# mika314/melonix

Measured on AMD Instinct MI355X. Metric: STFT+pitch+resynth frames/sec (48 kHz, 4096 FFT, 256 hop); % HBM roofline, higher is better.
Workload: dtype f32

## Files before the change

### melonix_amd/csrc/stft_core.h

```cpp
#pragma once
#include <stdint.h>
#include <type_traits>

#if defined(__HIPCC__)
#include <hip/hip_runtime.h>
#define MX_HD __host__ __device__ __forceinline__
namespace mx {
using cpx = float2;
}
#else
#define MX_HD inline __attribute__((always_inline))
namespace mx {
struct alignas(8) cpx {
  float x, y;
};
}
#endif

namespace mx {

#include "stft_consts.inc"

MX_HD cpx mk(float x, float y) {
  cpx r;
  r.x = x;
  r.y = y;
  return r;
}
MX_HD float fma_(float a, float b, float c) { return __builtin_fmaf(a, b, c); }
MX_HD cpx cadd(cpx a, cpx b) { return mk(a.x + b.x, a.y + b.y); }
MX_HD cpx csub(cpx a, cpx b) { return mk(a.x - b.x, a.y - b.y); }
MX_HD cpx cmul(cpx a, cpx b) { return mk(fma_(a.x, b.x, -(a.y * b.y)), fma_(a.x, b.y, a.y * b.x)); }
MX_HD float cnorm2(cpx a) { return fma_(a.x, a.x, a.y * a.y); }
MX_HD cpx cconj(cpx a) { return mk(a.x, -a.y); }
MX_HD cpx csel(bool c, cpx a, cpx b) { return mk(c ? a.x : b.x, c ? a.y : b.y); }
MX_HD float fast_sqrt(float x) {
#if defined(__HIP_DEVICE_COMPILE__)
  return __builtin_amdgcn_sqrtf(x);
#else
  return __builtin_sqrtf(x);
#endif
}
MX_HD constexpr int ilog2(int x) { return x <= 1 ? 0 : 1 + ilog2(x >> 1); }

}
#include "pk_math.h"
namespace mx {

template <int K>
MX_HD cpx mulw64(cpx a) {
  constexpr int k = ((K % 64) + 64) % 64;
  constexpr float h = 0.707106781187f;
  if constexpr (k == 0) return a;
  else if constexpr (k == 16) return mk(a.y, -a.x);
  else if constexpr (k == 32) return mk(-a.x, -a.y);
  else if constexpr (k == 48) return mk(-a.y, a.x);
  else if constexpr (k == 8) return mk(h * (a.x + a.y), h * (a.y - a.x));
  else if constexpr (k == 24) return mk(h * (a.y - a.x), -h * (a.x + a.y));
  else if constexpr (k == 40) return mk(-h * (a.x + a.y), h * (a.x - a.y));
  else if constexpr (k == 56) return mk(h * (a.x - a.y), h * (a.x + a.y));
  else {
    constexpr float c = kCos64[k], s = kSin64[k];
    return mk(fma_(a.x, c, a.y * s), fma_(a.y, c, -(a.x * s)));
  }
}

template <int K>
MX_HD void bfly_w64(cpx E, cpx O, cpx &out0, cpx &out1) {
  constexpr int k = ((K % 64) + 64) % 64;
  if constexpr (k == 0) {
    pk_bfly_1(E, O, out0, out1);
  } else if constexpr (k == 16) {
    pk_bfly_mi(E, O, out0, out1);
  } else if constexpr (k == 32) {
    pk_bfly_1(E, O, out1, out0);
  } else if constexpr (k == 48) {
    pk_bfly_mi(E, O, out1, out0);
  } else {
    pk_bfly_cs(E, O, mk(kCos64[k], kSin64[k]), out0, out1);
  }
}

template <int R, int Q>
struct Combine {
  static MX_HD void run(const cpx *E, const cpx *O, cpx *out) {
    bfly_w64<Q * 64 / R>(E[Q], O[Q], out[Q], out[Q + R / 2]);
    if constexpr (Q + 1 < R / 2) Combine<R, Q + 1>::run(E, O, out);
  }
};

template <int R>
struct Dft {
  static MX_HD void run(const cpx *in, cpx *out) {
    cpx e[R / 2], o[R / 2], E[R / 2], O[R / 2];
#pragma unroll
    for (int q = 0; q < R / 2; ++q) {
      e[q] = in[2 * q];
      o[q] = in[2 * q + 1];
    }
    Dft<R / 2>::run(e, E);
    Dft<R / 2>::run(o, O);
    Combine<R, 0>::run(E, O, out);
  }
};
template <>
struct Dft<2> {
  static MX_HD void run(const cpx *in, cpx *out) {
    pk_bfly_1(in[0], in[1], out[0], out[1]);
  }
};
template <>
struct Dft<1> {
  static MX_HD void run(const cpx *in, cpx *out) { out[0] = in[0]; }
};

template <int R, int S, int O0, bool CONJ>
struct DftTw {
  static MX_HD void run(const cpx *v, const cpx *w, cpx *out) {
    if constexpr (R == 2) {
      constexpr int i0 = O0, i1 = O0 + S;
      if constexpr (i0 == 0) pk_leaf0_tw<CONJ>(v[0], v[i1], w[i1], out[0], out[1]);
      else pk_leaf_tw<CONJ>(v[i0], w[i0], v[i1], w[i1], out[0], out[1]);
    } else {
      cpx E[R / 2], O[R / 2];
      DftTw<R / 2, 2 * S, O0, CONJ>::run(v, w, E);
      DftTw<R / 2, 2 * S, O0 + S, CONJ>::run(v, w, O);
      Combine<R, 0>::run(E, O, out);
    }
  }
};

template <int N_, int E_>
struct Plan {
  static constexpr int N = N_;
  static constexpr int M = N / 2;
  static constexpr int E = E_;
  static constexpr int T = M / E;
  static constexpr int R3 = E / 2;
  static constexpr int R1 = (N == 4096) ? 16 : 32;
  static constexpr int R2 = M / (R1 * R3);
  static constexpr int NS3 = R1 * R2;
  static constexpr int NB1 = E / R1;
  static constexpr int NB2 = E / R2;
  static constexpr int TW2 = (R2 - 1) * R1;
  static constexpr int TW3 = (R3 - 1) * NS3;
  static constexpr int L1 = ilog2(R1);
  static_assert(N == 4096 || N == 16384 || N == 32768, "supported FFT sizes");
  static_assert((N == 4096) ? E == 16 : E == 32, "supported points per thread");
  static_assert(R1 * R2 * R3 == M && R2 <= E && R1 <= E && T % 64 == 0, "radix plan must cover M");
};

template <class P>
MX_HD constexpr bool t1_padded() { return P::R1 == 32; }
template <class P>
MX_HD constexpr int t1_size() { return t1_padded<P>() ? P::M + P::M / 32 : P::M; }
template <class P>
MX_HD int t1_index(int i) {
  if constexpr (t1_padded<P>()) return i + (i >> 5);
  else return i ^ ((i >> P::L1) & 15);
}

struct alignas(4) f2u {
  float x, y;
};
template <bool ALIGNED8>
MX_HD cpx ld_pair(const float *base, int i) {
  const char *a = reinterpret_cast<const char *>(base) + (size_t)(4u * (unsigned)i);
  if constexpr (ALIGNED8) {
    return *reinterpret_cast<const cpx *>(a);
  } else {
    const f2u u = *reinterpret_cast<const f2u *>(a);
    return mk(u.x, u.y);
  }
}

MX_HD float ld_one(const float *base, int i) {
  return *reinterpret_cast<const float *>(reinterpret_cast<const char *>(base) + (size_t)(4u * (unsigned)i));
}

template <class P, int WSTEP, bool ALIGNED8>
MX_HD void load_frame(int t, cpx (&Y)[P::E], const float *x, const float *w) {
#pragma unroll
  for (int e = 0; e < P::E; ++e) {
    const int p = 2 * (t + P::T * e);
    cpx xs, ws;
    if constexpr (ALIGNED8 && WSTEP == 1) {
      xs = ld_pair<true>(x, p);
      ws = ld_pair<true>(w, p);
    } else {
      xs = ld_pair<false>(x, p);
      if constexpr (WSTEP == 1) {
        ws = ld_pair<false>(w, p);
      } else {
        const f2u wu = *reinterpret_cast<const f2u *>(w - p - 1);
        ws = mk(wu.y, wu.x);
      }
    }
    Y[e] = pk_mul(xs, ws);
  }
}

template <int T>
MX_HD constexpr float win_grow(int e) {
  return T == 64 ? kWinGrow64[e] : T == 128 ? kWinGrow128[e] : T == 256 ? kWinGrow256[e] : kWinGrow512[e];
}
template <class P, bool CLAMP = true>
MX_HD cpx geo_weight(cpx a0, int e) {
  constexpr float sc = 0.5f / (float)P::N;
  const float g = e == 0 ? 1.0f : win_grow<P::T>(e);
  const cpx w = e == 0 ? a0 : mk(a0.x * g, a0.y * g);
  if constexpr (!CLAMP) {
    return w;
  } else {
    const unsigned sb = __builtin_bit_cast(unsigned, sc), xb = __builtin_bit_cast(unsigned, w.x), yb = __builtin_bit_cast(unsigned, w.y);
    return mk(__builtin_bit_cast(float, xb < sb ? xb : sb), __builtin_bit_cast(float, yb < sb ? yb : sb));
  }
}
template <class P>
MX_HD int geo_clamped_slots(int hop) { return (hop + 2 * P::T - 1) / (2 * P::T); }
constexpr int kGeoTail = 2;
template <class P, bool ALIGNED8>
MX_HD void load_frame_geo(int t, cpx (&Y)[P::E], const float *x, const float *wb, int hop) {
  static_assert(P::T == 64 || P::T == 128 || P::T == 256 || P::T == 512, "growth table per T");
  static_assert(P::E <= 32, "growth table length");
  const cpx a0 = ld_pair<true>(wb, 2 * t);
  if (geo_clamped_slots<P>(hop) <= kGeoTail) {
#pragma unroll
    for (int e = 0; e < P::E; ++e) {
      const cpx xs = ld_pair<ALIGNED8>(x, 2 * (t + P::T * e));
      Y[e] = pk_mul(xs, e < P::E - kGeoTail ? geo_weight<P, false>(a0, e) : geo_weight<P, true>(a0, e));
    }
  } else {
#pragma unroll
    for (int e = 0; e < P::E; ++e) Y[e] = pk_mul(ld_pair<ALIGNED8>(x, 2 * (t + P::T * e)), geo_weight<P, true>(a0, e));
  }
}

template <class P>
MX_HD void apply_window_geo(int t, cpx (&Y)[P::E], const cpx (&xr)[P::E], const float *wb, int hop) {
  const cpx a0 = ld_pair<true>(wb, 2 * t);
  if (geo_clamped_slots<P>(hop) <= kGeoTail) {
#pragma unroll
    for (int e = 0; e < P::E; ++e)
      Y[e] = pk_mul(xr[e], e < P::E - kGeoTail ? geo_weight<P, false>(a0, e) : geo_weight<P, true>(a0, e));
  } else {
#pragma unroll
    for (int e = 0; e < P::E; ++e) Y[e] = pk_mul(xr[e], geo_weight<P, true>(a0, e));
  }
}

template <class P, bool ALIGNED8>
MX_HD void load_raw(int t, cpx (&xr)[P::E], const float *x) {
#pragma unroll
  for (int e = 0; e < P::E; ++e) {
    xr[e] = ld_pair<ALIGNED8>(x, 2 * (t + P::T * e));
  }
}
template <class P, int WSTEP, bool ALIGNED8>
MX_HD void apply_window(int t, cpx (&Y)[P::E], const cpx (&xr)[P::E], const float *w) {
#pragma unroll
  for (int e = 0; e < P::E; ++e) {
    const int p = 2 * (t + P::T * e);
    cpx ws;
    if constexpr (WSTEP == 1) {
      ws = ld_pair<ALIGNED8>(w, p);
    } else {
      const f2u wu = *reinterpret_cast<const f2u *>(w - p - 1);
      ws = mk(wu.y, wu.x);
    }
    Y[e] = pk_mul(xr[e], ws);
  }
}

template <class P>
MX_HD void pass1(const cpx (&Y)[P::E], cpx (&v)[P::E]) {
#pragma unroll
  for (int b = 0; b < P::NB1; ++b) {
    cpx in[P::R1], out[P::R1];
#pragma unroll
    for (int r = 0; r < P::R1; ++r) in[r] = Y[b + P::NB1 * r];
    Dft<P::R1>::run(in, out);
#pragma unroll
    for (int r = 0; r < P::R1; ++r) v[b * P::R1 + r] = out[r];
  }
}

template <class P, int HOP>
struct Slide {
  static constexpr int H = HOP / 2;
  static constexpr bool ok = (HOP > 0) && (HOP % 2 == 0) && (H % P::T == 0) && (2 * (H / P::T) <= P::E);
  static constexpr int D = ok ? H / P::T : 1;
};

template <class P, int HOP>
MX_HD void slide_edge(int t, const float *wtab, float inv_sc, cpx (&edge)[Slide<P, HOP>::D]) {
  using S = Slide<P, HOP>;
#pragma unroll
  for (int i = 0; i < S::D; ++i) {
    const int p = 2 * (t + P::T * (P::E - 2 * S::D + i));
    edge[i] = mk(wtab[p] * inv_sc, wtab[p + 1] * inv_sc);
  }
}

template <class P, int HOP>
MX_HD void slide_fetch(int t, const float *xe, cpx (&nx)[Slide<P, HOP>::D]) {
  using S = Slide<P, HOP>;
#pragma unroll
  for (int i = 0; i < S::D; ++i) nx[i] = *reinterpret_cast<const cpx *>(xe - HOP + 2 * (t + P::T * i));
}

template <class P, int HOP>
MX_HD void slide_step(cpx (&Y)[P::E], const cpx (&nx)[Slide<P, HOP>::D], const cpx (&edge)[Slide<P, HOP>::D],
                      float g, float sc) {
  using S = Slide<P, HOP>;
  const cpx gg = mk(g, g), ss = mk(sc, sc);
#pragma unroll
  for (int e = 0; e < P::E - 2 * S::D; ++e) Y[e] = pk_mul_xs(Y[e + S::D], gg);
#pragma unroll
  for (int i = 0; i < S::D; ++i) Y[P::E - 2 * S::D + i] = pk_mul(Y[P::E - S::D + i], edge[i]);
#pragma unroll
  for (int i = 0; i < S::D; ++i) Y[P::E - S::D + i] = pk_mul_xs(nx[i], ss);
}


template <class P>
struct Circ {
  static constexpr int W = 2 * P::T;
  static constexpr int CS = (P::T == 128) ? 4 : (P::T == 256) ? 3 : 2;
  static MX_HD bool ok(int hop) { return hop >= 1 && hop <= (CS - 1) * P::T && hop <= 2 * W; }
  static constexpr int slot(int k) { return (P::E - (CS - 1) + k) & (P::E - 1); }
};
template <class P>
struct CircGeo {
  int o;
  int s;
  int cr;
  int len;
};
template <class P>
MX_HD CircGeo<P> circ_geo(long long frame_end, int hop) {
  constexpr int W = Circ<P>::W;
  const long long start = frame_end - P::N;
  CircGeo<P> g;
  g.o = (int)(start & (long long)(W - 1));
  g.s = ((int)((start - hop) & (long long)(W - 1)) + hop) / W;
  g.len = 2 * hop;
  g.cr = (g.o - g.len) & (P::N - 1);
  return g;
}
template <class P>
MX_HD void circ_load_first(int t, cpx (&Y)[P::E], const float *xa, const float *w, int o) {
#pragma unroll
  for (int e = 0; e < P::E; ++e) {
    const int c2 = 2 * (t + P::T * e);
    const int q0 = (c2 - o) & (P::N - 1), q1 = (c2 + 1 - o) & (P::N - 1);
    Y[e] = mk(xa[q0] * w[q0], xa[q1] * w[q1]);
  }
}
template <class P>
MX_HD void circ_fetch(int t, const float *xs, const float *wt, const CircGeo<P> &g, float (&px)[2 * Circ<P>::CS],
                      float (&pw)[2 * Circ<P>::CS]) {
#pragma unroll
  for (int k = 0; k < Circ<P>::CS; ++k) {
    const int c2 = 2 * (t + P::T * Circ<P>::slot(k));
    int d0 = (c2 - g.cr) & (P::N - 1), d1 = (c2 + 1 - g.cr) & (P::N - 1);
    d0 = d0 < g.len ? d0 : g.len - 1;
    d1 = d1 < g.len ? d1 : g.len - 1;
    px[2 * k] = ld_one(xs, d0);
    px[2 * k + 1] = ld_one(xs, d1);
    pw[2 * k] = ld_one(wt, d0);
    pw[2 * k + 1] = ld_one(wt, d1);
  }
}
template <class P, int S>
MX_HD void circ_age(cpx (&Y)[P::E], cpx gg) {
  cpx head[S > 0 ? S : 1];
#pragma unroll
  for (int i = 0; i < S; ++i) head[i] = Y[i];
#pragma unroll
  for (int e = 0; e < P::E - S; ++e) Y[e] = pk_mul_xs(Y[e + S], gg);
#pragma unroll
  for (int i = 0; i < S; ++i) Y[P::E - S + i] = pk_mul_xs(head[i], gg);
}
template <class P>
MX_HD void circ_step(int t, cpx (&Y)[P::E], float decay, const CircGeo<P> &g, const float (&px)[2 * Circ<P>::CS],
                     const float (&pw)[2 * Circ<P>::CS]) {
  const cpx gg = mk(decay, decay);
  constexpr int SMAX = (Circ<P>::W - 1 + (Circ<P>::CS - 1) * P::T) / Circ<P>::W;
  static_assert(SMAX <= 2, "rotations by 0, 1 or 2 slots");
  if (g.s == 0) circ_age<P, 0>(Y, gg);
  else if (SMAX == 1 || g.s == 1) circ_age<P, 1>(Y, gg);
  else circ_age<P, 2>(Y, gg);
#pragma unroll
  for (int k = 0; k < Circ<P>::CS; ++k) {
    const int e = Circ<P>::slot(k);
    const int c2 = 2 * (t + P::T * e);
    const int d0 = (c2 - g.cr) & (P::N - 1), d1 = (c2 + 1 - g.cr) & (P::N - 1);
    const float n0 = px[2 * k] * pw[2 * k], n1 = px[2 * k + 1] * pw[2 * k + 1];
    Y[e] = mk(d0 < g.len ? n0 : Y[e].x, d1 < g.len ? n1 : Y[e].y);
  }
}


#if defined(__HIP_DEVICE_COMPILE__)
#define MX_LDS_ASM 1
typedef float mx_f2v __attribute__((ext_vector_type(2)));
template <int OFF>
__device__ __forceinline__ mx_f2v lds_rd64(uint32_t addr) {
  static_assert(OFF >= 0 && OFF < 163840, "LDS is 160 KiB");
  mx_f2v r;
  if constexpr (OFF < 65536) {
    asm volatile("ds_read_b64 %0, %1 offset:%2" : "=v"(r) : "v"(addr), "n"(OFF) : "memory");
  } else {
    const uint32_t hi = addr + (uint32_t)(OFF & ~65535);
    asm volatile("ds_read_b64 %0, %1 offset:%2" : "=v"(r) : "v"(hi), "n"(OFF & 65535) : "memory");
  }
  return r;
}
__device__ __forceinline__ uint32_t lds_addr(const void *p) {
  return (uint32_t)(uintptr_t)(const __attribute__((address_space(3))) void *)p;
}
template <int N>
__device__ __forceinline__ void lds_wait(mx_f2v (&q)[N]) {
  static_assert(N % 8 == 0, "tied in groups of 8");
  asm volatile("s_waitcnt lgkmcnt(0)" ::: "memory");
#pragma unroll
  for (int i = 0; i < N; i += 8)
    asm volatile("" : "+v"(q[i]), "+v"(q[i + 1]), "+v"(q[i + 2]), "+v"(q[i + 3]), "+v"(q[i + 4]),
                 "+v"(q[i + 5]), "+v"(q[i + 6]), "+v"(q[i + 7]));
}
#endif
template <int I, int N, class F>
MX_HD void static_for(F &&f) {
  if constexpr (I < N) {
    f(std::integral_constant<int, I>{});
    static_for<I + 1, N>(f);
  }
}

template <class P>
MX_HD void store_t1(int t, const cpx (&v)[P::E], cpx *lds) {
  if constexpr (t1_padded<P>()) {
    static_assert(P::R1 <= 32 && (P::T * P::R1) % 32 == 0, "T1 padding is one point per 32");
    cpx *const p = lds + (t * P::R1 + ((t * P::R1) >> 5));
#pragma unroll
    for (int b = 0; b < P::NB1; ++b) {
#pragma unroll
      for (int r = 0; r < P::R1; ++r) p[b * (P::T * P::R1 + P::T * P::R1 / 32) + r] = v[b * P::R1 + r];
    }
  } else {
    const unsigned B8 = (unsigned)((t * P::R1) ^ (t & 15)) << 3;
    char *const base = reinterpret_cast<char *>(lds);
#pragma unroll
    for (int r = 0; r < P::R1; ++r) {
      cpx *p = reinterpret_cast<cpx *>(base + (B8 ^ ((unsigned)r << 3)));
#pragma unroll
      for (int b = 0; b < P::NB1; ++b) p[b * P::T * P::R1] = v[b * P::R1 + r];
    }
  }
}

template <class P>
struct T1Read {
  static constexpr int S = P::M / P::R2;
  static constexpr int SP = t1_padded<P>() ? S + S / 32 : S;
  static constexpr int TP = t1_padded<P>() ? P::T + P::T / 32 : P::T;
  static constexpr int step = t1_padded<P>() ? 0 : ((S >> P::L1) & 15);
  static_assert(S % 32 == 0 && P::T % 32 == 0 && (step == 0 || step == 8), "T1 read is base(+alt base) + offset");
  static_assert(t1_padded<P>() || P::NB2 == 1, "the XOR layout's bases are written for one pass-2 butterfly per thread");
};

template <class P>
MX_HD void load_t1(int t, cpx (&v)[P::E], const cpx *lds) {
  using R = T1Read<P>;
  const int s1 = t1_index<P>(t);
#ifdef MX_LDS_ASM
  mx_f2v q[P::E];
  const uint32_t ae = lds_addr(lds + s1), ao = lds_addr(lds + (s1 ^ R::step));
  static_for<0, P::NB2>([&](auto bb) {
    constexpr int b = decltype(bb)::value;
    static_for<0, P::R2>([&](auto rr) {
      constexpr int r = decltype(rr)::value;
      q[b * P::R2 + r] = lds_rd64<(b * R::TP + r * R::SP) * 8>((r & 1) ? ao : ae);
    });
  });
  lds_wait(q);
#pragma unroll
  for (int i = 0; i < P::E; ++i) v[i] = mk(q[i].x, q[i].y);
#else
  const cpx *pe = lds + s1, *po = lds + (s1 ^ R::step);
#pragma unroll
  for (int b = 0; b < P::NB2; ++b) {
#pragma unroll
    for (int r = 0; r < P::R2; ++r) v[b * P::R2 + r] = ((r & 1) ? po : pe)[b * R::TP + r * R::SP];
  }
#endif
}

template <class P>
MX_HD void load_t1_tw2(int t, cpx (&v)[P::E], const cpx *lds, const cpx *ltw2, cpx (&w)[P::R2 - 1]) {
  static_assert(P::NB2 == 1 && P::E == P::R2 && P::E % 8 == 0, "one pass-2 butterfly per thread");
  using R = T1Read<P>;
  const int s1 = t1_index<P>(t);
#ifdef MX_LDS_ASM
  const uint32_t ae = lds_addr(lds + s1), ao = lds_addr(lds + (s1 ^ R::step));
  const uint32_t aw = lds_addr(ltw2 + (t & (P::R1 - 1)));
  mx_f2v q[2 * P::E];
  static_for<0, P::R2>([&](auto rr) {
    constexpr int r = decltype(rr)::value;
    q[r] = lds_rd64<r * R::SP * 8>((r & 1) ? ao : ae);
  });
  static_for<1, P::R2>([&](auto rr) {
    constexpr int r = decltype(rr)::value;
    q[P::E + r] = lds_rd64<(r - 1) * P::R1 * 8>(aw);
  });
  q[P::E] = mx_f2v{0.0f, 0.0f};
  lds_wait(q);
#pragma unroll
  for (int i = 0; i < P::E; ++i) v[i] = mk(q[i].x, q[i].y);
#pragma unroll
  for (int r = 1; r < P::R2; ++r) w[r - 1] = mk(q[P::E + r].x, q[P::E + r].y);
#else
  const cpx *pe = lds + s1, *po = lds + (s1 ^ R::step), *pw = ltw2 + (t & (P::R1 - 1));
#pragma unroll
  for (int r = 0; r < P::R2; ++r) v[r] = ((r & 1) ? po : pe)[r * R::SP];
#pragma unroll
  for (int r = 1; r < P::R2; ++r) w[r - 1] = pw[(r - 1) * P::R1];
#endif
}

template <class P>
MX_HD void pass2(int t, cpx (&v)[P::E], const cpx *tw2) {
#pragma unroll
  for (int b = 0; b < P::NB2; ++b) {
    const int j = t + P::T * b;
    const int k = j & (P::R1 - 1);
    cpx in[P::R2], w[P::R2], out[P::R2];
    w[0] = mk(1.0f, 0.0f);
#pragma unroll
    for (int r = 0; r < P::R2; ++r) in[r] = v[b * P::R2 + r];
#pragma unroll
    for (int r = 1; r < P::R2; ++r) {
      w[r] = tw2[(r - 1) * P::R1 + k];
    }
    DftTw<P::R2, 1, 0, false>::run(in, w, out);
#pragma unroll
    for (int r = 0; r < P::R2; ++r) v[b * P::R2 + r] = out[r];
  }
}

template <class P>
MX_HD void pass2_reg(cpx (&v)[P::E], const cpx (&w)[P::R2 - 1]) {
  static_assert(P::NB2 == 1, "one pass-2 butterfly per thread");
  cpx in[P::R2], ww[P::R2], out[P::R2];
  ww[0] = mk(1.0f, 0.0f);
#pragma unroll
  for (int r = 0; r < P::R2; ++r) in[r] = v[r];
#pragma unroll
  for (int r = 1; r < P::R2; ++r) ww[r] = w[r - 1];
  DftTw<P::R2, 1, 0, false>::run(in, ww, out);
#pragma unroll
  for (int r = 0; r < P::R2; ++r) v[r] = out[r];
}

template <class P>
MX_HD void store_t2(int t, const cpx (&v)[P::E], cpx *lds) {
#pragma unroll
  for (int b = 0; b < P::NB2; ++b) {
    const int j = t + P::T * b;
    const int k = j & (P::R1 - 1);
    const int base = (j - k) * P::R2 + k;
    cpx *p = lds + base;
#pragma unroll
    for (int r = 0; r < P::R2; ++r) p[r * P::R1] = v[b * P::R2 + r];
  }
}

template <class P>
MX_HD int k0p(int t) { return t; }
template <class P>
MX_HD int k0q(int t) { return t ? P::NS3 - t : P::NS3 / 2; }

template <class P>
MX_HD void load_t2(int t, cpx (&v)[P::E], const cpx *lds) {
  const int p = k0p<P>(t), q = k0q<P>(t);
#ifdef MX_LDS_ASM
  {
    const uint32_t pa = lds_addr(lds + p), qa = lds_addr(lds + q);
    mx_f2v w[P::E];
    static_for<0, P::R3>([&](auto rr) {
      constexpr int r = decltype(rr)::value;
      w[r] = lds_rd64<P::NS3 * r * 8>(pa);
      w[P::R3 + r] = lds_rd64<P::NS3 * r * 8>(qa);
    });
    lds_wait(w);
#pragma unroll
    for (int i = 0; i < P::E; ++i) v[i] = mk(w[i].x, w[i].y);
  }
#else
  const cpx *pp = lds + p, *qq = lds + q;
#pragma unroll
  for (int r = 0; r < P::R3; ++r) {
    v[r] = pp[P::NS3 * r];
    v[P::R3 + r] = qq[P::NS3 * r];
  }
#endif
}

template <class P>
MX_HD constexpr int q_index(int r) { return P::R3 + ((r + 1) & (P::R3 - 1)); }

template <class P>
MX_HD void fetch_tw3(int t, const cpx *tw3, cpx (&w)[P::R3 - 1]) {
  const int col = t ? t : P::NS3 / 2;
#pragma unroll
  for (int r = 1; r < P::R3; ++r) w[r - 1] = tw3[(r - 1) * P::NS3 + col];
}
template <class P>
MX_HD void fetch_tw3_bases(int t, const cpx *tw3, cpx (&wb)[6]) {
  static_assert(P::R3 == 16, "two-level pass-3 twiddles are written for radix 16");
  const int col = t ? t : P::NS3 / 2;
  constexpr int rr[6] = {1, 2, 3, 4, 8, 12};
#pragma unroll
  for (int i = 0; i < 6; ++i) wb[i] = tw3[(rr[i] - 1) * P::NS3 + col];
}
template <class P, bool MAY0>
MX_HD void pass3_reg(int t, cpx (&v)[P::E], const cpx (&w)[P::R3 - 1]);
template <class P, bool MAY0 = true>
MX_HD void pass3_bases(int t, cpx (&v)[P::E], const cpx (&wb)[6]) {
  cpx w[P::R3 - 1];
#pragma unroll
  for (int r = 1; r < P::R3; ++r) {
    const int hi = r >> 2, lo = r & 3;
    if (hi == 0) w[r - 1] = wb[lo - 1];
    else if (lo == 0) w[r - 1] = wb[2 + hi];
    else w[r - 1] = pk_cmul2(wb[2 + hi], wb[lo - 1]);
  }
  pass3_reg<P, MAY0>(t, v, w);
}
template <class P, bool MAY0 = true>
MX_HD void pass3_reg(int t, cpx (&v)[P::E], const cpx (&w)[P::R3 - 1]) {
  constexpr int R = P::R3;
  const bool t0 = MAY0 && (t == 0);
  cpx inp[R], inq[R], wp[R], wq[R], out[R];
  wp[0] = wq[0] = mk(1.0f, 0.0f);
#pragma unroll
  for (int r = 0; r < R; ++r) {
    inp[r] = v[r];
    inq[r] = v[R + r];
  }
#pragma unroll
  for (int r = 1; r < R; ++r) {
    wp[r] = csel(t0, mk(1.0f, 0.0f), w[r - 1]);
    wq[r] = w[r - 1];
  }
  DftTw<R, 1, 0, false>::run(inp, wp, out);
#pragma unroll
  for (int r = 0; r < R; ++r) v[r] = out[r];
  DftTw<R, 1, 0, true>::run(inq, wq, out);
#pragma unroll
  for (int r = 0; r < R; ++r) v[R + r] = out[r];
}

template <class P, int S>
struct PostSlot {
  static MX_HD void run(bool t0, const cpx (&v)[P::E], const cpx (&u)[P::R3], float (&mg)[P::E]) {
    constexpr int R = P::R3, H = R / 2;
    cpx A, B;
    if constexpr (S < H) {
      A = csel(t0, v[q_index<P>(S)], v[S]);
      B = v[q_index<P>(R - 1 - S)];
    } else {
      A = csel(t0, v[S - H], v[S]);
      B = csel(t0, v[(3 * H - S) & (R - 1)], v[q_index<P>(R - 1 - S)]);
    }
    const cpx n2 = pk_split_norm2(A, B, u[S]);
    mg[2 * S] = fast_sqrt(n2.x);
    mg[2 * S + 1] = fast_sqrt(n2.y);
    if constexpr (S == H) {
      const cpx z = v[H];
      const float m = fast_sqrt(cnorm2(z)) * 2.0f;
      mg[2 * S + 1] = t0 ? m : mg[2 * S + 1];
    }
    if constexpr (S + 1 < R) PostSlot<P, S + 1>::run(t0, v, u, mg);
  }
};

template <class P, bool MAY0 = true>
MX_HD void post(int t, const cpx (&v)[P::E], const cpx (&u)[P::R3], float (&mg)[P::E]) {
  PostSlot<P, 0>::run(MAY0 && t == 0, v, u, mg);
}

template <class P, int S>
struct PostFly {
  static MX_HD void run(cpx lo, cpx hi, cpx (&u)[P::R3]) {
    constexpr int k = ((32 / P::R3) * S) % 64;
    const cpx b = S < P::R3 / 2 ? lo : hi;
    if constexpr (k == 0) u[S] = b;
    else if constexpr (k == 16) u[S] = mk(b.y, -b.x);
    else u[S] = pk_rot_cs(b, mk(kCos64[k], kSin64[k]));
    if constexpr (S + 1 < P::R3) PostFly<P, S + 1>::run(lo, hi, u);
  }
};
template <class P>
MX_HD void post_bases(int t, const cpx *ubase, cpx &lo, cpx &hi) {
  if (t) {
    lo = ubase[t];
    hi = lo;
  } else {
    constexpr int k = 16 / P::R3;
    lo = mk(kSin64[k], kCos64[k]);
    hi = mk(-1.0f, 0.0f);
  }
}
template <class P, bool MAY0 = true>
MX_HD void post_fly(int t, const cpx (&v)[P::E], cpx lo, cpx hi, float (&mg)[P::E]) {
  cpx u[P::R3];
  PostFly<P, 0>::run(lo, MAY0 ? hi : lo, u);
  PostSlot<P, 0>::run(MAY0 && t == 0, v, u, mg);
}

template <class P, int S>
struct PostSlotC {
  static MX_HD void run(bool t0, const cpx (&v)[P::E], const cpx (&u)[P::R3], cpx (&X)[P::E]) {
    constexpr int R = P::R3, H = R / 2;
    cpx A, B;
    if constexpr (S < H) {
      A = csel(t0, v[q_index<P>(S)], v[S]);
      B = v[q_index<P>(R - 1 - S)];
    } else {
      A = csel(t0, v[S - H], v[S]);
      B = csel(t0, v[(3 * H - S) & (R - 1)], v[q_index<P>(R - 1 - S)]);
    }
    const cpx Sm = pk_add_cj(A, B);
    const cpx Dm = pk_sub_cj(A, B);
    const cpx D = pk_cmul<false>(Dm, u[S]);
    X[2 * S] = pk_sub(Sm, D);
    X[2 * S + 1] = cconj(pk_add(Sm, D));
    if constexpr (S == H) {
      const cpx z = v[H];
      X[2 * S + 1] = csel(t0, mk(2.0f * z.x, -2.0f * z.y), X[2 * S + 1]);
    }
    if constexpr (S + 1 < R) PostSlotC<P, S + 1>::run(t0, v, u, X);
  }
};
template <class P, bool MAY0 = true>
MX_HD void post_cplx(int t, const cpx (&v)[P::E], const cpx (&u)[P::R3], cpx (&X)[P::E]) {
  PostSlotC<P, 0>::run(MAY0 && t == 0, v, u, X);
}

template <class P>
MX_HD void out_bases(int t, int &lo, int &hi) {
  lo = t ? t : P::NS3 / 2;
  hi = t ? t : -(P::R3 / 2) * P::NS3;
}
template <class P>
MX_HD int out_bin(int t, int o) {
  int lo, hi;
  out_bases<P>(t, lo, hi);
  const int s = o >> 1;
  int k = (s < P::R3 / 2 ? lo : hi) + P::NS3 * s;
  if (o & 1) {
    k = P::M - k;
    if (k == P::M) k = P::M / 2;
  }
  return k;
}
template <class P>
MX_HD uint32_t band_mask(int t, int kmin, int kmax) {
  uint32_t m = 0;
#pragma unroll
  for (int o = 0; o < P::E; ++o) {
    const int k = out_bin<P>(t, o);
    m |= (k >= kmin && k <= kmax) ? (1u << o) : 0u;
  }
  return m;
}

template <class P, int S>
struct PostTw {
  static MX_HD void run(cpx lo, cpx hi, cpx (&u)[P::R3]) {
    u[S] = mulw64<(32 / P::R3) * S>(S < P::R3 / 2 ? lo : hi);
    if constexpr (S + 1 < P::R3) PostTw<P, S + 1>::run(lo, hi, u);
  }
};
template <class P>
MX_HD void post_twiddles(int t, const cpx *ubase, cpx (&u)[P::R3]) {
  cpx lo, hi;
  if (t) {
    lo = ubase[t];
    hi = lo;
  } else {
    constexpr int k = 16 / P::R3;
    lo = mk(kSin64[k], kCos64[k]);
    hi = mk(-1.0f, 0.0f);
  }
  PostTw<P, 0>::run(lo, hi, u);
}

}
```

### melonix_amd/csrc/stft_kernel_impl.h

```cpp
#pragma once
#include <hip/hip_runtime.h>

#include "colormap_core.h"
#include "kernels.h"
#include "stft_core.h"
#include "stft_tables.h"

#define MX_BARRIER() __syncthreads()

namespace mx {

template <bool MAXOP>
__device__ __forceinline__ unsigned wave_reduce_u32(unsigned k) {
  constexpr unsigned ident = MAXOP ? 0u : 0xffffffffu;
#define MX_DPP_STEP(CTRL, ROWS)                                                                      \
  {                                                                                                  \
    const unsigned o = (unsigned)__builtin_amdgcn_update_dpp((int)ident, (int)k, CTRL, ROWS, 0xf, false); \
    k = MAXOP ? (o > k ? o : k) : (o < k ? o : k);                                                   \
  }
  MX_DPP_STEP(0xB1, 0xf)
  MX_DPP_STEP(0x4E, 0xf)
  MX_DPP_STEP(0x141, 0xf)
  MX_DPP_STEP(0x140, 0xf)
  MX_DPP_STEP(0x142, 0xa)
  MX_DPP_STEP(0x143, 0xc)
#undef MX_DPP_STEP
  return (unsigned)__builtin_amdgcn_readlane((int)k, 63);
}
__device__ __forceinline__ unsigned long long wave_max_u64(unsigned long long k) {
  const unsigned hi = (unsigned)(k >> 32), lo = (unsigned)k;
  const unsigned mhi = wave_reduce_u32<true>(hi);
  const unsigned long long tie = __ballot(hi == mhi);
  unsigned mlo;
  if (__builtin_popcountll(tie) == 1) mlo = (unsigned)__builtin_amdgcn_readlane((int)lo, __builtin_ctzll(tie));
  else mlo = wave_reduce_u32<true>(hi == mhi ? lo : 0u);
  return ((unsigned long long)mhi << 32) | mlo;
}

template <int IMM, bool NT = true>
__device__ __forceinline__ void st_row_nt(const float *base, unsigned off, float x) {
  static_assert(IMM >= -4096 && IMM <= 4095, "global_store immediate offset");
#if defined(__HIP_DEVICE_COMPILE__)
  if constexpr (NT) asm volatile("global_store_dword %0, %1, %2 offset:%3 nt" : : "v"(off), "v"(x), "s"(base), "n"(IMM) : "memory");
  else asm volatile("global_store_dword %0, %1, %2 offset:%3" : : "v"(off), "v"(x), "s"(base), "n"(IMM) : "memory");
#endif
}

template <class P, int MODE, int HOP, int WPE, bool DEFER = false, bool PREFETCH = false, bool CMAP = false, bool DIRECT = false,
          bool CIRC = false>
__global__ __launch_bounds__(P::T) __attribute__((amdgpu_waves_per_eu(WPE, WPE)))
void stft_kernel(const StftArgs a0) {
  const StftArgs &a = a0;
  using C = P;
  constexpr int N = P::N;
  constexpr int NW = C::T / 64;
  constexpr int kRed = (NW > 1) ? ((NW + 1) / 2) * 2 : 0;
  constexpr bool kTw3Bases = (P::R3 == 16);
  constexpr int kTw2 = ((C::TW2 + 1) / 2) * 2;
  static_assert(P::R3 == 16 || P::R3 == 8, "twiddle placement per plan");
  static_assert(!DIRECT || (NW > 1 && !DEFER && !CMAP), "direct row stores: multi-wave, non-deferred plans");
  static_assert(!CIRC || (MODE != kRanges && HOP == 0 && !PREFETCH && !CMAP), "circular window: bulk modes");
  constexpr int IMG = t1_size<C>();
  __shared__ __attribute__((aligned(16))) float2 lds[IMG + kRed + (DEFER ? C::M / 2 : 0) + kTw2];
  float *const lout = reinterpret_cast<float *>(DEFER ? lds + IMG + kRed : lds);
  float2 *const ltw2 = lds + IMG + kRed + (DEFER ? C::M / 2 : 0);

  const int t_ = threadIdx.x;
  const bool wave0 = __builtin_amdgcn_readfirstlane(t_) < 64;
  cpx u[kTw3Bases ? 1 : P::R3];
  cpx ulo;
  cpx w3r[kTw3Bases ? 1 : P::R3 - 1], w3base[6];
  if constexpr (kTw3Bases) {
    cpx uhi_unused;
    post_bases<P>(t_, a.ubase, ulo, uhi_unused);
    fetch_tw3_bases<P>(t_, a.tw3, w3base);
  } else {
    post_twiddles<P>(t_, a.ubase, *reinterpret_cast<cpx(*)[P::R3]>(&u));
    fetch_tw3<P>(t_, a.tw3, *reinterpret_cast<cpx(*)[P::R3 - 1]>(&w3r));
  }
  const uint32_t bmask_ = band_mask<P>(t_, a.kmin, a.kmax);
  uint32_t umask = 0;
#pragma unroll
  for (int o = 0; o < P::E; ++o) umask |= (__ballot((bmask_ >> o) & 1u) != 0ull) ? (1u << o) : 0u;
  umask = __builtin_amdgcn_readfirstlane(umask);
  constexpr bool kSlide = (MODE == kBulkAligned) && (HOP > 0) && Slide<P, (HOP > 0 ? HOP : 2)>::ok;
  constexpr int SD = Slide<P, (HOP > 0 ? HOP : 2)>::D;
  constexpr float kSc = 0.5f / (float)N;
  for (int i = t_; i < C::TW2; i += C::T) ltw2[i] = a.tw2[i];
  MX_BARRIER();

  unsigned lb = blockIdx.x;
  {
    const unsigned nb = gridDim.x, xcd = lb & 7u, q = nb >> 3, r = nb & 7u;
    lb = (xcd < r ? xcd * (q + 1) : r * (q + 1) + (xcd - r) * q) + (lb >> 3);
  }
  const int64_t f0 = (int64_t)lb * a.frames_per_block;
  const int64_t f1 = (f0 + a.frames_per_block < a.count) ? f0 + a.frames_per_block : a.count;

  cpx Y[P::E];
  cpx edge[SD], nx[SD];
  if constexpr (kSlide) {
    const int64_t e0 = (a.first_frame + f0 + 1) * (int64_t)HOP;
    if (f0 < f1) load_frame<P, 1, true>(t_, Y, a.audio + MX_AUDIO_PAD + (e0 - N), a.wtab);
    slide_edge<P, HOP>(t_, a.wtab, 2.0f * (float)N, edge);
  }

  unsigned long long *const red = reinterpret_cast<unsigned long long *>(lds + IMG);
  auto flush_pitch = [&](int64_t fr, int tt) {
    if (a.pitch && tt == 0) {
      unsigned long long b = red[0];
#pragma unroll
      for (int i = 1; i < NW; ++i) b = red[i] > b ? red[i] : b;
      mx_pitch p;
      p.bin = 0x7fffffff - (int)(unsigned)(b & 0xffffffffull);
      p.mag = __uint_as_float((unsigned)(b >> 32));
      a.pitch[fr] = p;
    }
  };
  const bool want_rows = a.mags != nullptr || (CMAP && a.rgb != nullptr);
  auto flush_row = [&](int64_t fr, int tt) {
    if (want_rows) {
      using f32x4 = float __attribute__((ext_vector_type(4)));
      const f32x4 *l4 = reinterpret_cast<const f32x4 *>(lout) + tt;
      f32x4 *row4 = reinterpret_cast<f32x4 *>(a.mags + (size_t)fr * (size_t)(N / 2)) + tt;
      f32x4 q[C::M / 4 / C::T];
#pragma unroll
      for (int i = 0; i < C::M / 4 / C::T; ++i) q[i] = l4[C::T * i];
      if (!CMAP || a.mags) {
#pragma unroll
        for (int i = 0; i < C::M / 4 / C::T; ++i) {
          __builtin_nontemporal_store(q[i], &row4[C::T * i]);
        }
      }
      if constexpr (CMAP) {
        if (a.rgb) {
          uint32_t *trow = reinterpret_cast<uint32_t *>(a.rgb + (size_t)fr * (size_t)(N / 2) * 3) + 3 * tt;
#pragma unroll 1
          for (int i = 0; i < C::M / 4 / C::T; ++i) {
            uint32_t w3[3];
            texel4(q[i].x, q[i].y, q[i].z, q[i].w, a.cmap_k, w3);
            uint32_t *o = trow + 3 * C::T * i;
            o[0] = w3[0];
            o[1] = w3[1];
            o[2] = w3[2];
          }
        }
      }
    }
  };

  auto frame_ptrs = [&](int64_t fr, int zo, const float *&x, const float *&w) {
    if constexpr (MODE == kRanges) {
      const int s = a.ranges[2 * fr], e = a.ranges[2 * fr + 1];
      const bool outside = (e <= 0) || ((int64_t)e - N >= a.n);
      x = outside ? a.audio : a.audio + MX_AUDIO_PAD + ((int64_t)e - N);
      int64_t d0 = (int64_t)N - ((int64_t)e - (int64_t)s);
      d0 = d0 < (int64_t)(N - 1 - kWOff) ? (int64_t)(N - 1 - kWOff) : d0;
      d0 = d0 > (int64_t)(kWDmax + kWTail) ? (int64_t)(kWDmax + kWTail) : d0;
      w = a.wext + kWOff + d0;
    } else {
      const int64_t e = (a.first_frame + fr + 1) * (int64_t)a.hop;
      x = a.audio + MX_AUDIO_PAD + (e - N);
      w = a.wtab + zo;
    }
  };
  float cpx_[2 * Circ<P>::CS], cpw_[2 * Circ<P>::CS];
  if constexpr (CIRC) {
    if (f0 < f1) {
      const int64_t pe = (a.first_frame + f0 + 1) * (int64_t)a.hop;
      circ_load_first<P>(t_, Y, a.audio + MX_AUDIO_PAD + (pe - N), a.wtab, circ_geo<P>(pe, a.hop).o);
    }
  }
  cpx xr[(PREFETCH && !kSlide) ? P::E : 1];
  if constexpr (PREFETCH && !kSlide) {
    if (f0 < f1) {
      const float *x0;
      const float *w0;
      frame_ptrs(f0, 0, x0, w0);
      load_raw<P, (MODE == kBulkAligned)>(t_, xr, x0);
    }
  }

  for (int64_t f = f0; f < f1; ++f) {
    int t = t_;
    unsigned bmask = bmask_;
    int zoff = 0;
    asm volatile("" : "+v"(t), "+v"(bmask), "+s"(zoff));
    int out_lo, out_hi;
    out_bases<P>(t, out_lo, out_hi);

    if constexpr (CIRC) {
      if (f > f0) {
        const int64_t pe = (a.first_frame + f + 1) * (int64_t)a.hop;
        const CircGeo<P> geo = circ_geo<P>(pe, a.hop);
        circ_fetch<P>(t, a.audio + MX_AUDIO_PAD + (pe - 2 * (int64_t)a.hop), a.wtab + zoff + (N - 2 * a.hop), geo, cpx_, cpw_);
        circ_step<P>(t, Y, a.decay, geo, cpx_, cpw_);
      }
    } else if constexpr (kSlide) {
      if (f > f0) slide_step<P, HOP>(Y, nx, edge, a.decay, kSc);
      if (f + 1 < f1) slide_fetch<P, HOP>(t, a.audio + MX_AUDIO_PAD + (a.first_frame + f + 2) * (int64_t)HOP, nx);
    } else {
      const float *x;
      const float *w;
      frame_ptrs(f, zoff, x, w);
      if constexpr (PREFETCH) {
        if constexpr (MODE == kRanges) apply_window<P, -1, false>(t, Y, xr, w);
        else apply_window_geo<P>(t, Y, xr, a.wtab + N + zoff, a.hop);
      } else if constexpr (MODE == kRanges) {
        load_frame<P, -1, false>(t, Y, x, w);
      } else {
        load_frame_geo<P, (MODE == kBulkAligned)>(t, Y, x, a.wtab + N + zoff, a.hop);
      }
    }

    cpx v[P::E];
    pass1<P>(Y, v);
    constexpr bool kTw2Batch = (P::NB2 == 1);
    store_t1<P>(t, v, lds);
    MX_BARRIER();
    if constexpr (DEFER || DIRECT) {
      if (f > f0) flush_pitch(f - 1, t);
    }
    if constexpr (kTw2Batch) {
      cpx w2[P::R2 - 1];
      load_t1_tw2<P>(t, v, lds, ltw2, w2);
      if constexpr (DEFER) {
        if (f > f0) flush_row(f - 1, t);
      }
      MX_BARRIER();
      pass2_reg<P>(v, w2);
    } else {
      load_t1<P>(t, v, lds);
      if constexpr (DEFER) {
        if (f > f0) flush_row(f - 1, t);
      }
      MX_BARRIER();
      pass2<P>(t, v, ltw2);
    }
    store_t2<P>(t, v, lds);
    MX_BARRIER();
    load_t2<P>(t, v, lds);
    MX_BARRIER();
    float mg[P::E];
    if (NW == 1 || wave0) {
      if constexpr (kTw3Bases) {
        pass3_bases<P, true>(t, v, w3base);
        post_fly<P, true>(t, v, ulo, csel(t == 0, mk(-1.0f, 0.0f), ulo), mg);
      } else {
        pass3_reg<P, true>(t, v, *reinterpret_cast<cpx(*)[P::R3 - 1]>(&w3r));
        post<P, true>(t, v, *reinterpret_cast<cpx(*)[P::R3]>(&u), mg);
      }
    } else {
      if constexpr (kTw3Bases) {
        pass3_bases<P, false>(t, v, w3base);
        post_fly<P, false>(t, v, ulo, ulo, mg);
      } else {
        pass3_reg<P, false>(t, v, *reinterpret_cast<cpx(*)[P::R3 - 1]>(&w3r));
        post<P, false>(t, v, *reinterpret_cast<cpx(*)[P::R3]>(&u), mg);
      }
    }

    if constexpr (PREFETCH && !kSlide) {
      if (f + 1 < f1) {
        const float *xn;
        const float *wn;
        frame_ptrs(f + 1, zoff, xn, wn);
        load_raw<P, (MODE == kBulkAligned)>(t, xr, xn);
      }
    }

    unsigned long long best = 0ull;
    if (a.pitch) {
      const unsigned klo = 0x7fffffffu - (unsigned)out_lo, khi = 0x7fffffffu - (unsigned)out_hi;
      const unsigned nlo = 0x7fffffffu - (unsigned)(C::M - out_lo), nhi = 0x7fffffffu - (unsigned)(C::M - out_hi);
#pragma unroll
      for (int s = 0; s < C::R3; ++s) {
        constexpr int H = C::R3 / 2;
        if (!((umask >> (2 * s)) & 3u)) continue;
        const unsigned b0 = (s < H ? klo : khi) - (unsigned)(C::NS3 * s);
        unsigned b1 = (s < H ? nlo : nhi) + (unsigned)(C::NS3 * s);
        if (s == H) b1 = (t == 0) ? 0x7fffffffu - (unsigned)(C::M / 2) : b1;
        const unsigned v0 = (unsigned)((int)(bmask << (31 - 2 * s)) >> 31);
        const unsigned v1 = (unsigned)((int)(bmask << (31 - (2 * s + 1))) >> 31);
        const unsigned long long k0 = ((unsigned long long)(__float_as_uint(mg[2 * s]) & v0) << 32) | (b0 & v0);
        const unsigned long long k1 = ((unsigned long long)(__float_as_uint(mg[2 * s + 1]) & v1) << 32) | (b1 & v1);
        best = k0 > best ? k0 : best;
        best = k1 > best ? k1 : best;
      }
      best = wave_max_u64(best);
      if constexpr (NW > 1) {
        if ((t & 63) == 0) red[t >> 6] = best;
      }
    }

    if constexpr (DIRECT) {
      if (want_rows) {
        const float *row = a.mags + (size_t)f * (size_t)(N / 2);
        constexpr int H = C::R3 / 2;
        constexpr int STEP = 4 * C::NS3;
        constexpr int G = 8192 / STEP;
        static_assert((STEP == 4096 || STEP == 2048) && H % G == 0, "slot groups share an offset through the store's immediate");
        const unsigned blo = 4u * (unsigned)out_lo, bhi = 4u * (unsigned)(out_hi + C::NS3 * H);
        const unsigned nlo = 4u * (unsigned)(C::M - out_lo), nhi = 4u * (unsigned)(C::M - out_hi - C::NS3 * H);
        static_for<0, C::R3>([&](auto ss) {
          constexpr int s = decltype(ss)::value;
          constexpr int sl = s < H ? s : s - H;
          constexpr int su = (sl & ~(G - 1)) + G / 2, sd = (sl & ~(G - 1)) + G / 2 - 1;
          const unsigned o0 = (s < H ? blo : bhi) + (unsigned)(su * STEP);
          unsigned o1 = (s < H ? nlo : nhi) - (unsigned)(sd * STEP);
          if constexpr (s == H) {
            o1 = (t == 0) ? (unsigned)(4 * (C::M / 2)) + (unsigned)((sl - sd) * STEP) : o1;
          }
          st_row_nt<(sl - su) * STEP>(row, o0, mg[2 * s]);
          st_row_nt<-(sl - sd) * STEP, false>(row, o1, mg[2 * s + 1]);
        });
      }
    } else if (want_rows) {
      float *plo = lout + out_lo, *phi = lout + out_hi;
      float *mlo = lout + (C::M - out_lo), *mhi = lout + (C::M - out_hi);
#pragma unroll
      for (int s = 0; s < C::R3; ++s) {
        constexpr int H = C::R3 / 2;
        (s < H ? plo : phi)[C::NS3 * s] = mg[2 * s];
        if (s == H) (t == 0 ? lout + C::M / 2 : mhi - C::NS3 * H)[0] = mg[2 * s + 1];
        else (s < H ? mlo : mhi)[-C::NS3 * s] = mg[2 * s + 1];
      }
    }
    if constexpr (!DEFER && !DIRECT) {
      if (want_rows) {
        MX_BARRIER();
        flush_row(f, t);
        MX_BARRIER();
      } else {
        MX_BARRIER();
      }
      if constexpr (NW > 1) {
        flush_pitch(f, t);
      } else if (a.pitch && t == 0) {
        mx_pitch p;
        p.bin = 0x7fffffff - (int)(unsigned)(best & 0xffffffffull);
        p.mag = __uint_as_float((unsigned)(best >> 32));
        a.pitch[f] = p;
      }
    }
  }
  if constexpr (DEFER || DIRECT) {
    if (f0 < f1) {
      MX_BARRIER();
      flush_pitch(f1 - 1, t_);
      if constexpr (DEFER) flush_row(f1 - 1, t_);
    }
  }
}


}
```

### melonix_amd/csrc/stft_kernels.hip

```cpp
#include <hip/hip_runtime.h>

#include "kernels.h"
#include "stft_kernel_impl.h"

namespace mx {

namespace {

template <class P>
struct Tune {
  static constexpr bool TWO_WAVE = (P::E == 16);
  static constexpr int WPE = TWO_WAVE ? 3 : 2;
  static constexpr bool PREFETCH = (P::E == 32);
  static constexpr bool slides(int hop) {
    return P::N == 4096 ? (hop == 256 || hop == 512) : P::N == 16384 ? (hop == 512 || hop == 1024) : hop == 1024;
  }
  static constexpr bool DIRECT = (P::N >= 16384);
  static constexpr bool CIRC = (P::N >= 16384);
  static constexpr bool DEFER = TWO_WAVE;
};

template <class P, int HOP>
bool try_slide(const StftArgs &b, dim3 grid, dim3 block, hipStream_t s) {
  if constexpr (Slide<P, HOP>::ok && Tune<P>::slides(HOP)) {
    if (b.hop != HOP) return false;
    hipLaunchKernelGGL((stft_kernel<P, kBulkAligned, HOP, Tune<P>::WPE, Tune<P>::DEFER, false, false, Tune<P>::DIRECT>),
                       grid, block, 0, s, b);
    return true;
  } else {
    return false;
  }
}

template <class P>
bool try_circ(const StftArgs &b, dim3 grid, dim3 block, hipStream_t s) {
  if constexpr (!Tune<P>::CIRC) {
    return false;
  } else {
    if (!Circ<P>::ok(b.hop)) return false;
    hipLaunchKernelGGL((stft_kernel<P, kBulkAny, 0, Tune<P>::WPE, Tune<P>::DEFER, false, false, Tune<P>::DIRECT, true>),
                       grid, block, 0, s, b);
    return true;
  }
}

template <class P>
hipError_t launch_plan(int mode, const StftArgs &a, hipStream_t s) {
  if (a.count <= 0) return hipSuccess;
  const int g = a.frames_per_block > 0 ? a.frames_per_block : 1;
  const int64_t blocks = (a.count + g - 1) / g;
  if (blocks > 0x7fffffffLL) return hipErrorInvalidValue;
  StftArgs b = a;
  b.frames_per_block = g;
  const dim3 grid((unsigned)blocks), block(P::T);
  constexpr int W = Tune<P>::WPE;
  constexpr bool DF = Tune<P>::DEFER, PF = Tune<P>::PREFETCH, DR = Tune<P>::DIRECT;
  switch (mode) {
    case kBulkAligned:
      if (!(try_slide<P, 256>(b, grid, block, s) || try_slide<P, 512>(b, grid, block, s) ||
            try_slide<P, 1024>(b, grid, block, s) || try_circ<P>(b, grid, block, s)))
        hipLaunchKernelGGL((stft_kernel<P, kBulkAligned, 0, W, DF, PF, false, DR>), grid, block, 0, s, b);
      break;
    case kBulkAny:
      if (try_circ<P>(b, grid, block, s)) break;
      hipLaunchKernelGGL((stft_kernel<P, kBulkAny, 0, W, DF, PF, false, DR>), grid, block, 0, s, b); break;
    case kRanges:
      if (a.rgb) hipLaunchKernelGGL((stft_kernel<P, kRanges, 0, (W > 2 ? 2 : W), DF, false, true>), grid, block, 0, s, b);
      else hipLaunchKernelGGL((stft_kernel<P, kRanges, 0, W, DF, false, false, DR>), grid, block, 0, s, b);
      break;
    default: return hipErrorInvalidValue;
  }
  return hipGetLastError();
}

}

int stft_points_per_thread(int N) { return N == 4096 ? kPlan4096E : 32; }

int stft_frames_per_block_cap(int N, int mode, int hop) {
  if (N == 32768 && mode != kRanges && Tune<Plan<32768, 32>>::CIRC && !Tune<Plan<32768, 32>>::slides(hop) &&
      Circ<Plan<32768, 32>>::ok(hop))
    return 32;
  return N == 32768 ? 8 : (N == 4096 ? 32 : 16);
}

hipError_t launch_stft(int N, int mode, const StftArgs &a, hipStream_t s) {
  switch (N) {
    case 4096: return launch_plan<Plan<4096, kPlan4096E>>(mode, a, s);
    case 16384: return launch_plan<Plan<16384, 32>>(mode, a, s);
    case 32768: return launch_plan<Plan<32768, 32>>(mode, a, s);
  }
  return hipErrorInvalidValue;
}

}
```

Baseline: 327.9 million.

## Fuse pitch argmax into deferred row flush for two-wave sliding kernels

Adds a ROWPICK path for the deferred two-wave sliding STFT kernel. It drops the per-element pitch argmax scan over butterfly outputs and instead computes the argmax while flushing the magnitude row from LDS. Each wave takes the other wave's half of the row and scans only the groups that overlap the band. A cross-wave reduction and barrier run only when the band spans both halves. The path is used only when both the magnitude and pitch outputs are requested, and it adds extra bookkeeping and a conditional barrier.

```diff
diff --git a/melonix_amd/csrc/stft_core.h b/melonix_amd/csrc/stft_core.h
--- a/melonix_amd/csrc/stft_core.h
+++ b/melonix_amd/csrc/stft_core.h
@@ -777,6 +777,49 @@
   return m;
 }
 
+template <class P>
+struct RowPick {
+  static constexpr int G = P::M / 4 / P::T;
+  static constexpr int S = 4 * P::T;
+  static constexpr int W = 4 * 64;
+  static_assert(P::T == 128 && 4 * G <= 32, "two wavefronts swap halves; a lane's band bits fit a word");
+  static MX_HD int group(int tt) { return tt ^ 64; }
+  static MX_HD uint32_t lane_mask(int g, int kmin, int kmax) {
+    uint32_t m = 0;
+#pragma unroll
+    for (int o = 0; o < 4 * G; ++o) {
+      const int k = 4 * g + S * (o >> 2) + (o & 3);
+      m |= (k >= kmin && k <= kmax) ? (1u << o) : 0u;
+    }
+    return m;
+  }
+  static MX_HD uint32_t wave_groups(int wave, int kmin, int kmax) {
+    uint32_t m = 0;
+#pragma unroll
+    for (int i = 0; i < G; ++i) {
+      const int lo = W * (wave ^ 1) + S * i;
+      m |= (kmin <= lo + W - 1 && kmax >= lo) ? (1u << i) : 0u;
+    }
+    return m;
+  }
+  static MX_HD bool takes_part(int wave, int kmin, int kmax) {
+    const bool mine = wave_groups(wave, kmin, kmax) != 0, other = wave_groups(wave ^ 1, kmin, kmax) != 0;
+    return mine || (wave == 1 && !other);
+  }
+  static MX_HD bool both(int kmin, int kmax) { return wave_groups(0, kmin, kmax) != 0 && wave_groups(1, kmin, kmax) != 0; }
+  static MX_HD unsigned key0(int g, int i) { return 0x7fffffffu - (unsigned)(4 * g + S * i); }
+  static MX_HD unsigned long long scan4(unsigned long long best, float x0, float x1, float x2, float x3, uint32_t m4, unsigned k0) {
+    const float x[4] = {x0, x1, x2, x3};
+#pragma unroll
+    for (int j = 0; j < 4; ++j) {
+      const unsigned v = (unsigned)((int)(m4 << (31 - j)) >> 31);
+      const unsigned long long k = ((unsigned long long)(__builtin_bit_cast(unsigned, x[j]) & v) << 32) | ((k0 - (unsigned)j) & v);
+      best = k > best ? k : best;
+    }
+    return best;
+  }
+};
+
 template <class P, int S>
 struct PostTw {
   static MX_HD void run(cpx lo, cpx hi, cpx (&u)[P::R3]) {
diff --git a/melonix_amd/csrc/stft_kernel_impl.h b/melonix_amd/csrc/stft_kernel_impl.h
--- a/melonix_amd/csrc/stft_kernel_impl.h
+++ b/melonix_amd/csrc/stft_kernel_impl.h
@@ -47,7 +47,7 @@
 }
 
 template <class P, int MODE, int HOP, int WPE, bool DEFER = false, bool PREFETCH = false, bool CMAP = false, bool DIRECT = false,
-          bool CIRC = false>
+          bool CIRC = false, bool ROWPICK = false>
 __global__ __launch_bounds__(P::T) __attribute__((amdgpu_waves_per_eu(WPE, WPE)))
 void stft_kernel(const StftArgs a0) {
   const StftArgs &a = a0;
@@ -60,6 +60,7 @@
   static_assert(P::R3 == 16 || P::R3 == 8, "twiddle placement per plan");
   static_assert(!DIRECT || (NW > 1 && !DEFER && !CMAP), "direct row stores: multi-wave, non-deferred plans");
   static_assert(!CIRC || (MODE != kRanges && HOP == 0 && !PREFETCH && !CMAP), "circular window: bulk modes");
+  static_assert(!ROWPICK || (DEFER && NW == 2 && MODE == kBulkAligned && HOP > 0 && !CMAP), "row pick: the deferred two-wave sliding kernels");
   constexpr int IMG = t1_size<C>();
   __shared__ __attribute__((aligned(16))) float2 lds[IMG + kRed + (DEFER ? C::M / 2 : 0) + kTw2];
   float *const lout = reinterpret_cast<float *>(DEFER ? lds + IMG + kRed : lds);
@@ -78,11 +79,21 @@
     post_twiddles<P>(t_, a.ubase, *reinterpret_cast<cpx(*)[P::R3]>(&u));
     fetch_tw3<P>(t_, a.tw3, *reinterpret_cast<cpx(*)[P::R3 - 1]>(&w3r));
   }
-  const uint32_t bmask_ = band_mask<P>(t_, a.kmin, a.kmax);
-  uint32_t umask = 0;
-#pragma unroll
-  for (int o = 0; o < P::E; ++o) umask |= (__ballot((bmask_ >> o) & 1u) != 0ull) ? (1u << o) : 0u;
-  umask = __builtin_amdgcn_readfirstlane(umask);
+  uint32_t bmask_, umask = 0, pk_groups = 0;
+  bool pk_take = false, pk_both = false;
+  if constexpr (ROWPICK) {
+    using RP = RowPick<P>;
+    bmask_ = RP::lane_mask(RP::group(t_), a.kmin, a.kmax);
+    const int wv = wave0 ? 0 : 1;
+    pk_groups = RP::wave_groups(wv, a.kmin, a.kmax);
+    pk_take = a.pitch != nullptr && RP::takes_part(wv, a.kmin, a.kmax);
+    pk_both = a.pitch != nullptr && RP::both(a.kmin, a.kmax);
+  } else {
+    bmask_ = band_mask<P>(t_, a.kmin, a.kmax);
+#pragma unroll
+    for (int o = 0; o < P::E; ++o) umask |= (__ballot((bmask_ >> o) & 1u) != 0ull) ? (1u << o) : 0u;
+    umask = __builtin_amdgcn_readfirstlane(umask);
+  }
   constexpr bool kSlide = (MODE == kBulkAligned) && (HOP > 0) && Slide<P, (HOP > 0 ? HOP : 2)>::ok;
   constexpr int SD = Slide<P, (HOP > 0 ? HOP : 2)>::D;
   constexpr float kSc = 0.5f / (float)N;
@@ -118,11 +129,13 @@
     }
   };
   const bool want_rows = a.mags != nullptr || (CMAP && a.rgb != nullptr);
-  auto flush_row = [&](int64_t fr, int tt) {
+  auto flush_row = [&](int64_t fr, int tt, uint32_t lm) {
     if (want_rows) {
       using f32x4 = float __attribute__((ext_vector_type(4)));
-      const f32x4 *l4 = reinterpret_cast<const f32x4 *>(lout) + tt;
-      f32x4 *row4 = reinterpret_cast<f32x4 *>(a.mags + (size_t)fr * (size_t)(N / 2)) + tt;
+      int wg = tt;
+      if constexpr (ROWPICK) wg = RowPick<P>::group(tt);
+      const f32x4 *l4 = reinterpret_cast<const f32x4 *>(lout) + wg;
+      f32x4 *row4 = reinterpret_cast<f32x4 *>(a.mags + (size_t)fr * (size_t)(N / 2)) + wg;
       f32x4 q[C::M / 4 / C::T];
 #pragma unroll
       for (int i = 0; i < C::M / 4 / C::T; ++i) q[i] = l4[C::T * i];
@@ -130,6 +143,28 @@
 #pragma unroll
         for (int i = 0; i < C::M / 4 / C::T; ++i) {
           __builtin_nontemporal_store(q[i], &row4[C::T * i]);
+        }
+      }
+      if constexpr (ROWPICK) {
+        if (pk_take) {
+          using RP = RowPick<P>;
+          unsigned long long best = 0ull;
+#pragma unroll
+          for (int i = 0; i < RP::G; ++i) {
+            if (!((pk_groups >> i) & 1u)) continue;
+            best = RP::scan4(best, q[i].x, q[i].y, q[i].z, q[i].w, lm >> (4 * i), RP::key0(wg, i));
+          }
+          best = wave_max_u64(best);
+          if ((tt & 63) == 0) {
+            if (pk_both) {
+              red[tt >> 6] = best;
+            } else {
+              mx_pitch p;
+              p.bin = 0x7fffffff - (int)(unsigned)(best & 0xffffffffull);
+              p.mag = __uint_as_float((unsigned)(best >> 32));
+              a.pitch[fr] = p;
+            }
+          }
         }
       }
       if constexpr (CMAP) {
@@ -218,21 +253,28 @@
     constexpr bool kTw2Batch = (P::NB2 == 1);
     store_t1<P>(t, v, lds);
     MX_BARRIER();
-    if constexpr (DEFER || DIRECT) {
+    if constexpr ((DEFER || DIRECT) && !ROWPICK) {
       if (f > f0) flush_pitch(f - 1, t);
     }
     if constexpr (kTw2Batch) {
       cpx w2[P::R2 - 1];
+      if constexpr (ROWPICK) {
+        if (f > f0) flush_row(f - 1, t, bmask);
+      }
       load_t1_tw2<P>(t, v, lds, ltw2, w2);
-      if constexpr (DEFER) {
-        if (f > f0) flush_row(f - 1, t);
+      if constexpr (DEFER && !ROWPICK) {
+        if (f > f0) flush_row(f - 1, t, bmask);
       }
       MX_BARRIER();
+      if constexpr (ROWPICK) {
+        if (pk_both && f > f0) flush_pitch(f - 1, t);
+      }
       pass2_reg<P>(v, w2);
     } else {
+      static_assert(!ROWPICK, "row pick: one pass-2 butterfly per thread");
       load_t1<P>(t, v, lds);
       if constexpr (DEFER) {
-        if (f > f0) flush_row(f - 1, t);
+        if (f > f0) flush_row(f - 1, t, bmask);
       }
       MX_BARRIER();
       pass2<P>(t, v, ltw2);
@@ -270,7 +312,7 @@
     }
 
     unsigned long long best = 0ull;
-    if (a.pitch) {
+    if (!ROWPICK && a.pitch) {
       const unsigned klo = 0x7fffffffu - (unsigned)out_lo, khi = 0x7fffffffu - (unsigned)out_hi;
       const unsigned nlo = 0x7fffffffu - (unsigned)(C::M - out_lo), nhi = 0x7fffffffu - (unsigned)(C::M - out_hi);
 #pragma unroll
@@ -329,7 +371,7 @@
     if constexpr (!DEFER && !DIRECT) {
       if (want_rows) {
         MX_BARRIER();
-        flush_row(f, t);
+        flush_row(f, t, 0u);
         MX_BARRIER();
       } else {
         MX_BARRIER();
@@ -347,8 +389,14 @@
   if constexpr (DEFER || DIRECT) {
     if (f0 < f1) {
       MX_BARRIER();
-      flush_pitch(f1 - 1, t_);
-      if constexpr (DEFER) flush_row(f1 - 1, t_);
+      if constexpr (!ROWPICK) flush_pitch(f1 - 1, t_);
+      if constexpr (DEFER) flush_row(f1 - 1, t_, bmask_);
+      if constexpr (ROWPICK) {
+        if (pk_both) {
+          MX_BARRIER();
+          flush_pitch(f1 - 1, t_);
+        }
+      }
     }
   }
 }
diff --git a/melonix_amd/csrc/stft_kernels.hip b/melonix_amd/csrc/stft_kernels.hip
--- a/melonix_amd/csrc/stft_kernels.hip
+++ b/melonix_amd/csrc/stft_kernels.hip
@@ -24,6 +24,12 @@
 bool try_slide(const StftArgs &b, dim3 grid, dim3 block, hipStream_t s) {
   if constexpr (Slide<P, HOP>::ok && Tune<P>::slides(HOP)) {
     if (b.hop != HOP) return false;
+    if constexpr (Tune<P>::DEFER) {
+      if (b.mags != nullptr && b.pitch != nullptr) {
+        hipLaunchKernelGGL((stft_kernel<P, kBulkAligned, HOP, Tune<P>::WPE, true, false, false, false, false, true>), grid, block, 0, s, b);
+        return true;
+      }
+    }
     hipLaunchKernelGGL((stft_kernel<P, kBulkAligned, HOP, Tune<P>::WPE, Tune<P>::DEFER, false, false, Tune<P>::DIRECT>),
                        grid, block, 0, s, b);
     return true;
```

Measured after the change: 331.0 million (median of 6 runs). No clear change (+0.9%).
